# junyanz/interactive-deep-colorization

Hardware: NVIDIA H100
Metric: net_forward images/sec @256x256 (higher is better)
Workload: dtype f16x2-split operands, f32 accumulate (ab within 1e-3 of the f32 reference)

## Files before the change

### interactive_deep_colorization_b200/csrc/idc_api.cu

```cuda
#include <math.h>
#include <stdarg.h>
#include <stdio.h>
#include <string.h>

#include <algorithm>
#include <cmath>

#include "idc_internal.h"

using namespace idc;

struct idc_ctx : public idc::Ctx {};

namespace {

int fail(Ctx* c, int code, const char* fmt, ...) {
  char buf[512];
  va_list ap;
  va_start(ap, fmt);
  vsnprintf(buf, sizeof(buf), fmt, ap);
  va_end(ap);
  if (c) c->err = buf;
  return code;
}
// ... 680 lines not shown
    CUDA_TRY(c, mark());
  }
  const bool fused = !c->simt && !(c->flags & IDC_FLAG_KEEP_CONV10);
  if (!fused) CUDA_TRY(c, launch_out_head(c, n, out_ab, st));
  if (out_dist && !forked) {
    CUDA_TRY(c, launch_softmax529(c, n, out_dist, st));
    CUDA_TRY(c, click_tail(c, n, st));
    pdl_break(c);
  }
  if (out_rgb) {
    CUDA_TRY(c, launch_lab2rgb(c, n, c->H, c->W, L, 50.0f, out_ab, out_rgb, st, out_abq));
    c->launch_count++;
  }
  if (forked) {
    CUDA_TRY(c, cudaStreamWaitEvent(st, c->side->ev_join.get(), 0));
    pdl_break(c);
  }
  CUDA_TRY(c, mark());
  pdl_break(c);
  c->last_n = n;
  return IDC_OK;
}

int check_forward_args(Ctx* c, int n, int h, int w, const void* L, const void* ab, const void* mask, const void* glob,
                       const void* out_ab, const void* out_dist, bool resident_l_ok = false, bool hints_ok = false) {
  if (!c->weights_ready) return fail(c, IDC_ERR_STATE, "idc_forward before idc_finalize_weights");
  if (n < 1 || n > c->max_n) return fail(c, IDC_ERR_ARG, "n=%d outside [1,%d]", n, c->max_n);
  if (h != c->H || w != c->W) return fail(c, IDC_ERR_ARG, "geometry %dx%d != ctx geometry %dx%d", h, w, c->H, c->W);
  const bool hint_mode = hints_ok && !ab && !mask;
  if ((!L && !resident_l_ok) || ((!ab || !mask) && !hint_mode) || !out_ab)
    return fail(c, IDC_ERR_ARG, "null L/ab/mask/out_ab");
  if (out_dist && !c->dist) return fail(c, IDC_ERR_ARG, "out_dist requires IDC_FLAG_DIST");
  if (glob && !c->glob) return fail(c, IDC_ERR_ARG, "glob requires IDC_FLAG_GLOBAL_HINTS");
  return IDC_OK;
}

}

extern "C" {

const char* idc_version(void) { return "idc_b200 0.2 sm_90a (wgmma split-fp16 + fp32 simt engines)"; }

int idc_create(int device, int max_n, int h, int w, unsigned flags, idc_ctx** out) {
  if (!out) return IDC_ERR_ARG;
  *out = nullptr;
  if (max_n < 1 || h < 8 || w < 8 || (h % 8) || (w % 8)) return IDC_ERR_ARG;
  int ndev = 0;
  if (cudaGetDeviceCount(&ndev) != cudaSuccess || device < 0 || device >= ndev) return IDC_ERR_CUDA;
  cudaDeviceProp prop;
  if (cudaGetDeviceProperties(&prop, device) != cudaSuccess) return IDC_ERR_CUDA;
  if (prop.major != 9 || prop.minor != 0) return IDC_ERR_UNSUPPORTED;
  if (cudaSetDevice(device) != cudaSuccess) return IDC_ERR_CUDA;
  std::unique_ptr<idc_ctx> c(new idc_ctx());
  c->dev = device; c->num_sms = prop.multiProcessorCount; c->max_n = max_n; c->H = h; c->W = w; c->flags = flags;
  c->simt = flags & IDC_FLAG_ENGINE_SIMT;
  c->fast = (flags & IDC_FLAG_FAST_FP16) && !c->simt;
  c->dist = flags & IDC_FLAG_DIST;
  c->glob = flags & IDC_FLAG_GLOBAL_HINTS;
  c->caffe313 = flags & IDC_FLAG_CAFFE313;
  build_plan(c.get());
  int rc = alloc_workspace(c.get());
  if (rc != IDC_OK) {
    fprintf(stderr, "idc_create: %s\n", c->err.c_str());
    return rc;
  }
  *out = c.release();
  return IDC_OK;
}

int idc_set_option(idc_ctx* c, const char* name, int value) {
  if (!c || !name) return IDC_ERR_ARG;
  if (!strncmp(name, "act_exp.", 8)) {
    auto it = c->buf_index.find(name + 8);
    if (it == c->buf_index.end() || c->bufs[it->second].H == 0) return fail(c, IDC_ERR_KEY, "no activation '%s'", name + 8);
    if (value < kActExpMin || value > kActExpMax)
      return fail(c, IDC_ERR_ARG, "%s = %d outside [%d, %d]", name, value, kActExpMin, kActExpMax);
    if (c->weights_adopted)
      return fail(c, IDC_ERR_STATE, "%s must be set before the weights are packed (idc_finalize_weights)", name);
    c->act_exp_override[name + 8] = value;
    return IDC_OK;
  }
  struct { const char* n; int* v; } tab[] = {
      {"halo", &c->opt.halo}, {"pairs", &c->opt.pairs}, {"mt", &c->opt.mt},
      {"chunk_kb", &c->opt.chunk_kb}, {"split_k", &c->opt.split_k}, {"host_pipe", &c->opt.host_pipe},
      {"pdl", &c->opt.pdl}, {"tanh_scale", &c->opt.tanh_scale}, {"side_dist", &c->opt.side_dist},
      {"conv1_1_umma", &c->opt.conv1_1_umma}};
  for (auto& t : tab)
    if (!strcmp(t.n, name)) {
      *t.v = value;
      if (c->weights_adopted && strcmp(name, "host_pipe") && strcmp(name, "tanh_scale") && strcmp(name, "side_dist") && strcmp(name, "conv1_1_umma")) {
        CUDA_TRY(c, cudaSetDevice(c->dev));
        CUDA_TRY(c, cudaDeviceSynchronize());
        int rc = plan_engines(c);
        if (rc != IDC_OK) return rc;
      }
      c->graph_exec.reset();
      return IDC_OK;
    }
  return fail(c, IDC_ERR_KEY, "unknown option '%s'", name);
}

int idc_load_tensor(idc_ctx* c, const char* key, const void* data, int dtype, int ndim, const int64_t* dims) {
  if (!c || !key || !data || ndim < 0 || ndim > 8 || (ndim && !dims)) return fail(c, IDC_ERR_ARG, "bad load_tensor args");
  HostTensor t;
  size_t count = 1;
  for (int i = 0; i < ndim; ++i) {
    if (dims[i] < 0) return fail(c, IDC_ERR_ARG, "negative dim");
    t.dims.push_back(dims[i]);
    count *= (size_t)dims[i];
  }
  t.data.resize(count);
  switch (dtype) {
    case IDC_F32: memcpy(t.data.data(), data, count * sizeof(float)); break;
    case IDC_F64: for (size_t i = 0; i < count; ++i) t.data[i] = (float)((const double*)data)[i]; break;
    case IDC_I64: for (size_t i = 0; i < count; ++i) t.data[i] = (float)((const int64_t*)data)[i]; break;
    default: return fail(c, IDC_ERR_ARG, "unknown dtype %d", dtype);
  }
  c->raw[key] = std::move(t);
  c->weights_ready = c->weights_adopted = false;
  return IDC_OK;
}

int idc_reserve_weights(idc_ctx* c) {
  if (!c) return IDC_ERR_ARG;
  CUDA_TRY(c, cudaSetDevice(c->dev));
  if (!c->arena.get()) {
    c->arena_bytes = layout_arena(c, nullptr);
    CUDA_TRY(c, cudaMalloc(c->arena.put(), c->arena_bytes));
    layout_arena(c, c->arena.get());
  }
  return IDC_OK;
}

int idc_finalize_weights(idc_ctx* c) {
  if (!c) return IDC_ERR_ARG;
  int rc = idc_reserve_weights(c);
  if (rc != IDC_OK) return rc;
  std::vector<char> host(c->arena_bytes, 0);
  rc = pack_weights(c, host.data());
  if (rc != IDC_OK) return rc;
  if (c->caffe313) {
    const HostTensor* pts = find(c, "caffe.pts_in_hull");
    if (!check_dims(pts, {313, 2})) return fail(c, IDC_ERR_KEY, "missing/bad caffe.pts_in_hull [313,2]");
    CUDA_TRY(c, cudaMemcpy(c->pts313.get(), pts->data.data(), sizeof(float) * 626, cudaMemcpyHostToDevice));
  }
  CUDA_TRY(c, cudaMemcpy(c->arena.get(), host.data(), c->arena_bytes, cudaMemcpyHostToDevice));
  return idc_adopt_weights(c);
}

int idc_adopt_weights(idc_ctx* c) {
  if (!c || !c->arena.get()) return fail(c, IDC_ERR_STATE, "no arena");
  CUDA_TRY(c, cudaSetDevice(c->dev));
  CUDA_TRY(c, cudaMemcpy(c->h_w11.w, c->w11, sizeof(c->h_w11.w), cudaMemcpyDeviceToHost));
  CUDA_TRY(c, cudaMemcpy(c->h_w11.b, c->b11, sizeof(c->h_w11.b), cudaMemcpyDeviceToHost));
  std::vector<int> exps(c->bufs.size());
  CUDA_TRY(c, cudaMemcpy(exps.data(), c->act_exp, exps.size() * sizeof(int), cudaMemcpyDeviceToHost));
  for (size_t i = 0; i < exps.size(); ++i) c->bufs[i].exp = exps[i];
  if (!c->simt) CUDA_TRY(c, conv1_1_umma_pack(c));
  int rc = plan_engines(c);
  if (rc != IDC_OK) return rc;
  c->raw.clear();
  c->weights_adopted = true;
  c->graph_exec.reset();
  return IDC_OK;
}

int idc_weights_arena(idc_ctx* c, void** dev_ptr, size_t* bytes) {
// ... 799 lines not shown
```

### interactive_deep_colorization_b200/csrc/idc_internal.h

```cpp
#pragma once
#include <cuda.h>
#include <cuda_fp16.h>
#include <cuda_runtime.h>
#include <stdint.h>

#include <map>
#include <memory>
#include <string>
#include <utility>
#include <vector>

#include "../../include/idc_b200.h"

namespace idc {

template <typename H, auto Release>
class Owner {
 public:
  Owner() = default;
  Owner(Owner&& o) noexcept { std::swap(h_, o.h_); }
  Owner& operator=(Owner&& o) noexcept { std::swap(h_, o.h_); return *this; }
  ~Owner() { reset(); }
  H get() const { return h_; }
  H* put() { reset(); return &h_; }
// ... 15 lines not shown

constexpr int kActExpRef = 7;
constexpr int kActExpBound = 11;
constexpr int kActExpCal = 10;
constexpr int kActExpMin = -24, kActExpMax = 24;
constexpr unsigned kRangeInputBit = 31;
constexpr unsigned kF16MaxBits = 0x7BFFu;
constexpr int kInExp = 6;
constexpr float kInScale = 64.0f;

struct Tap {
  int src;
  int ky, kx;
  int ty, tx;
};

struct ActBuf {
  std::string name;
  int H = 0, W = 0, C = 0;
  int exp = 0;
  DevMem<void> p0, p1;
};

struct Epilogue {
  float* bias = nullptr;
  float* scale = nullptr;
  float* shift = nullptr;
  int act = ACT_NONE;
  bool has_bn = false;
  bool gadd = false;
};

struct SrcDesc {
  int buf = -1;
  int s = 1;
  int cin = 0;
};

enum OpKind { OP_CONV = 0, OP_UP = 1, OP_CLASS = 2, OP_HYPER = 3 };

struct UmmaPlan;
struct UmmaPlanFree { void operator()(UmmaPlan* p) const; };

struct ConvOp {
  std::string name;
  int kind = OP_CONV;
  std::string wkey[kMaxSrc];
  bool src_deconv[kMaxSrc] = {false, false, false, false, false, false};
  int src_k[kMaxSrc] = {3, 3, 3, 3, 3, 3};
  std::string bnkey;
  int nsrc = 1;
  SrcDesc src[kMaxSrc];
  int ncls = 1;
  int ntaps = 0;
  Tap taps[kMaxCls][kMaxTaps];
  int Hl = 0, Wl = 0;
  int out_buf = -1;
  int os = 1;
  int cout = 0, cout_pad = 0;
  int K = 0;
  Epilogue epi;
  bool fuse_out_head = false;
  bool out_f32 = false;
  float* out_f32_ptr = nullptr;
  float* w_simt = nullptr;
  __half* w_hi = nullptr;
  __half* w_lo = nullptr;
  int bn_tile = 0, hbox = 0, wbox = 0;
  std::unique_ptr<UmmaPlan, UmmaPlanFree> umma_plan;
  double flops_per_image = 0;
};

struct Conv11Weights {
  float w[36 * 64];
  float b[64];
};

struct Options {
  int halo = 1;
  int pairs = 0;
  int mt = -1;
  int chunk_kb = -1;
  int split_k = -1;
  int host_pipe = 1;
  int pdl = 1;
  int conv1_1_umma = 1;
  int side_dist = 1;
  int tanh_scale = 110;
};

struct HostTensor {
  std::vector<float> data;
  std::vector<int64_t> dims;
};

struct HostStaging {
  DevMem<float> d_in, d_out; HostMem<float> h_in, h_out;
  DevMem<uint8_t> d_rgb; HostMem<uint8_t> h_rgb;
  DevMem<char> d_small; HostMem<char> h_small;
};
struct AbqStaging { DevMem<double> d_abq; HostMem<double> h_abq; };
struct HintBlock { HostMem<char> h_hints; DevMem<char> d_hints; };
struct ClickBlock {
  HostMem<int> h_click; int* d_click = nullptr;
  DevMem<char> d_clickout; HostMem<char> h_clickout;
};
struct SideBranch { Stream s_side, s_click; Event ev_fork, ev_join, ev_click[2]; };
struct HostPipeStreams { Stream s_in, s_out; Event ev_in[8], ev_out[8]; };

struct Ctx {
  int dev = 0;
  int num_sms = 0;
  int max_n = 0, H = 0, W = 0;
  unsigned flags = 0;
  Options opt;
  bool simt = false, fast = false, dist = false, glob = false;
  std::map<std::string, HostTensor> raw;
  std::vector<ActBuf> bufs;
  std::map<std::string, int> buf_index;
  std::vector<ConvOp> ops;
  DevMem<char> arena;
  size_t arena_bytes = 0;
  int* act_exp = nullptr;
  std::map<std::string, int> act_exp_override;
  std::map<std::string, double> act_range;
  DevMem<unsigned> d_absmax;
  bool weights_ready = false;
  bool weights_adopted = false;
  float* w11 = nullptr;
  float* b11 = nullptr;
  Conv11Weights h_w11;
  DevMem<uint8_t> w11_umma;
  float* wout = nullptr;
  float* bout = nullptr;
  float* gw[4] = {nullptr, nullptr, nullptr, nullptr};
  float* gb[4] = {nullptr, nullptr, nullptr, nullptr};
  float* gscale[4] = {nullptr, nullptr, nullptr, nullptr};
  float* gshift[4] = {nullptr, nullptr, nullptr, nullptr};
  DevMem<float> gvec;
  DevMem<float> gtmp;
  DevMem<float> logits;
  DevMem<float> logits313;
  bool caffe313 = false;
  DevMem<float> pts313;
  DevMem<float> splitk_ws; size_t splitk_ws_floats = 0;
  DevMem<int> splitk_counters; int splitk_max_tiles = 0;
  bool dbg_graph_timing = false;
  Event dbg_ev[2];
  float dbg_graph_ms = 0.f;
  HostMem<int> h_err;
  int* d_err = nullptr;
  unsigned* d_range = nullptr;
  std::unique_ptr<HostStaging> stage;
  std::unique_ptr<AbqStaging> abq;
  Stream own_stream;
  std::unique_ptr<HostPipeStreams> pipe;
  std::unique_ptr<SideBranch> side;
  int image_n = 0;
  std::unique_ptr<HintBlock> hints;
  int graph_captures = 0;
  GraphExec graph_exec;
  const void* graph_ptrs[8] = {nullptr};
  float graph_maskcent = 0.f;
  int launch_count = 0;
  int graph_launches = 0;
  bool chain = false;
// ... 209 lines not shown
```

### interactive_deep_colorization_b200/csrc/idc_umma.cu

```cuda
#include <stdio.h>
#include <stdlib.h>

#include "idc_internal.h"

namespace idc {

constexpr int kBM = 128;
constexpr int kBK = 64;
constexpr int kThreads = 384;
constexpr int kProdRegs = 40;
constexpr int kMathRegs = 232;
constexpr int kMathThreads = 256;

struct UmmaParams {
  const CUtensorMap* amaps;
  const int4* kblk;
  int nkb, ncls;
  int chunk_kb;
  int split_k;
  float* ws;
  int* counters;
  int n_img, tiles_y, tiles_x, n_tiles_n, total_tiles;
  int hbox, wbox, wshift;
  int Hl, Wl, cout_pad;
  const float* bias;
  const float* scale;
  const float* shift;
  const float* gadd;
  int gadd_ld;
  float gadd_mult;
  int act;
  __half* out_hi;
  __half* out_lo;
  int Hout, Wout, Cout, os;
  float* out_f32;
  int out_ld;
  const float* wout;
  const float* bout;
  float* out_ab;
  float out_mult;
  int* err;
  unsigned* range;
  unsigned range_bit;
  int n_amaps;
  int max_ctas;
  int img0;
};

__device__ __forceinline__ uint32_t smem_u32(const void* p) { return (uint32_t)__cvta_generic_to_shared(p); }

__device__ __forceinline__ void mbar_init(uint32_t bar, uint32_t count) {
  asm volatile("mbarrier.init.shared::cta.b64 [%0], %1;" ::"r"(bar), "r"(count));
}
__device__ __forceinline__ void mbar_expect_tx(uint32_t bar, uint32_t bytes) {
  asm volatile("mbarrier.arrive.expect_tx.shared::cta.b64 _, [%0], %1;" ::"r"(bar), "r"(bytes) : "memory");
}
__device__ __forceinline__ void mbar_arrive(uint32_t bar) {
  asm volatile("mbarrier.arrive.shared::cta.b64 _, [%0];" ::"r"(bar) : "memory");
}
__device__ __forceinline__ uint32_t mbar_try_wait(uint32_t bar, uint32_t parity) {
  uint32_t ok;
  asm volatile(
      "{\n\t.reg .pred p;\n\t"
      "mbarrier.try_wait.parity.shared::cta.b64 p, [%1], %2;\n\t"
      "selp.u32 %0, 1, 0, p;\n\t}"
      : "=r"(ok)
      : "r"(bar), "r"(parity)
      : "memory");
  return ok;
}
__device__ __noinline__ void mbar_timeout(int* err, int code) {
  if (err) {
    atomicExch(err, code);
    __threadfence_system();
  }
  __trap();
}
__device__ __forceinline__ void mbar_wait(uint32_t bar, uint32_t parity, int* err, int code) {
  if (mbar_try_wait(bar, parity)) return;
  const long long t0 = clock64();
  while (!mbar_try_wait(bar, parity)) {
    if (clock64() - t0 > 6000000000LL) mbar_timeout(err, code);
  }
}

__device__ __forceinline__ bool elect_one() {
  uint32_t pred;
  asm volatile(
      "{\n\t.reg .pred p;\n\t"
      "elect.sync _|p, 0xffffffff;\n\t"
      "selp.u32 %0, 1, 0, p;\n\t}"
      : "=r"(pred));
  return pred != 0;
}

__device__ __forceinline__ void tma_load_4d(uint32_t dst, const void* tmap, uint32_t bar, int c0, int c1, int c2,
                                            int c3) {
  asm volatile(
      "cp.async.bulk.tensor.4d.shared::cluster.global.mbarrier::complete_tx::bytes [%0], [%1, {%3, %4, %5, %6}], [%2];"
      ::"r"(dst), "l"(tmap), "r"(bar), "r"(c0), "r"(c1), "r"(c2), "r"(c3)
      : "memory");
}
__device__ __forceinline__ void tma_load_2d(uint32_t dst, const void* tmap, uint32_t bar, int c0, int c1) {
  asm volatile(
      "cp.async.bulk.tensor.2d.shared::cluster.global.mbarrier::complete_tx::bytes [%0], [%1, {%3, %4}], [%2];"
      ::"r"(dst), "l"(tmap), "r"(bar), "r"(c0), "r"(c1)
      : "memory");
}

__device__ __forceinline__ void tma_load_2d_mc(uint32_t dst, const void* tmap, uint32_t bar, int c0, int c1) {
  asm volatile(
      "cp.async.bulk.tensor.2d.shared::cluster.global.mbarrier::complete_tx::bytes.multicast::cluster"
      " [%0], [%1, {%3, %4}], [%2], %5;"
      ::"r"(dst), "l"(tmap), "r"(bar), "r"(c0), "r"(c1), "h"((uint16_t)3)
      : "memory");
}
__device__ __forceinline__ uint32_t cluster_ctarank() {
  uint32_t r;
  asm volatile("mov.u32 %0, %%cluster_ctarank;" : "=r"(r));
  return r;
}
__device__ __forceinline__ void cluster_sync_all() {
  asm volatile("barrier.cluster.arrive.release.aligned;" ::: "memory");
  asm volatile("barrier.cluster.wait.acquire.aligned;" ::: "memory");
}
__device__ __forceinline__ void mbar_arrive_remote(uint32_t local_bar, uint32_t rank) {
  asm volatile(
      "{\n\t.reg .b32 ra;\n\t"
      "mapa.shared::cluster.u32 ra, %0, %1;\n\t"
      "mbarrier.arrive.release.cluster.shared::cluster.b64 _, [ra];\n\t}"
      ::"r"(local_bar), "r"(rank)
      : "memory");
}

__device__ __forceinline__ void pdl_wait() { asm volatile("griddepcontrol.wait;" ::: "memory"); }
__device__ __forceinline__ void pdl_launch_dependents() { asm volatile("griddepcontrol.launch_dependents;" ::: "memory"); }
__device__ __forceinline__ void prefetch_tmap(const void* tmap) {
  asm volatile("prefetch.tensormap [%0];" ::"l"(tmap) : "memory");
}

__device__ __forceinline__ void st_shared_u32(uint32_t addr, uint32_t v) {
  asm volatile("st.shared.b32 [%0], %1;" ::"r"(addr), "r"(v) : "memory");
}
__device__ __forceinline__ uint4 ld_shared_v4(uint32_t addr) {
  uint4 v;
  asm volatile("ld.shared.v4.b32 {%0, %1, %2, %3}, [%4];" : "=r"(v.x), "=r"(v.y), "=r"(v.z), "=r"(v.w) : "r"(addr));
  return v;
}

__device__ __forceinline__ void wgmma_fence() { asm volatile("wgmma.fence.sync.aligned;" ::: "memory"); }
__device__ __forceinline__ void wgmma_commit() { asm volatile("wgmma.commit_group.sync.aligned;" ::: "memory"); }
template <int N>
__device__ __forceinline__ void wgmma_wait() { asm volatile("wgmma.wait_group.sync.aligned %0;" ::"n"(N) : "memory"); }
template <int R>
__device__ __forceinline__ void wgmma_reg_fence(float (&d)[R]) {
#pragma unroll
  for (int i = 0; i < R; ++i) asm volatile("" : "+f"(d[i])::"memory");
}

__device__ __forceinline__ void wgmma_n64(float (&d)[32], uint64_t adesc, uint64_t bdesc, uint32_t accumulate) {
  asm volatile(
      "{\n\t.reg .pred p;\n\t"
      "setp.ne.b32 p, %34, 0;\n\t"
      "wgmma.mma_async.sync.aligned.m64n64k16.f32.f16.f16 "
// ... 19 lines not shown
  if constexpr (BN == 128) wgmma_n128(d, adesc, bdesc, accumulate);
  else wgmma_n64(d, adesc, bdesc, accumulate);
}

__device__ __forceinline__ uint64_t make_sw128_desc(uint32_t smem_addr, uint32_t sbo = 1024u) {
  uint64_t d = 0;
  d |= (uint64_t)((smem_addr >> 4) & 0x3FFFu);
  d |= (uint64_t)1 << 16;
  d |= (uint64_t)(sbo >> 4) << 32;
  d |= (uint64_t)1 << 62;
  return d;
}

__device__ __forceinline__ uint32_t pack_f16x2_sat(float a, float b) {
  uint32_t r;
  asm("cvt.rn.satfinite.f16x2.f32 %0, %1, %2;" : "=r"(r) : "f"(b), "f"(a));
  return r;
}
__device__ __forceinline__ uint32_t lo_f16x2(float a, float b, uint32_t hw) {
  const float2 hf = __half22float2(*reinterpret_cast<const __half2*>(&hw));
  return pack_f16x2_sat(a - hf.x, b - hf.y);
}
__device__ __forceinline__ uint32_t habs_max2(uint32_t m, uint32_t w) {
  const __half2 r = __hmax2(*reinterpret_cast<const __half2*>(&m), __habs2(*reinterpret_cast<const __half2*>(&w)));
  return *reinterpret_cast<const uint32_t*>(&r);
}
__device__ __forceinline__ bool f16_top(uint32_t m) {
  return ((m & 0xFFFFu) >= kF16MaxBits) | ((m >> 16) >= kF16MaxBits);
}

__device__ __forceinline__ void split_h(float v, __half& hi, __half& lo) {
  v = fminf(fmaxf(v, -65504.f), 65504.f);
  hi = __float2half_rn(v);
  lo = __float2half_rn(v - __half2float(hi));
}

__device__ __forceinline__ int frag_col(int i, int lane) { return 8 * (i >> 2) + 2 * (lane & 3) + (i & 1); }

constexpr int kHaloW = 10, kHaloH = 18;
constexpr int kHaloPlane = (kHaloW * kHaloH * 128 + 1023) / 1024 * 1024;


template <int BN, int MT, int CG, bool SPLIT, bool HALO>
struct SmemPlan {
  static constexpr int kABytes = MT * kBM * kBK * 2;
  static constexpr int kAStage = HALO ? 0 : kABytes;
  static constexpr int kBBytes = BN * kBK * 2;
  static constexpr int kStageBytes = (SPLIT ? 2 : 1) * (kAStage + kBBytes);
  static constexpr int kHaloSlot = (SPLIT ? 2 : 1) * kHaloPlane;
  static constexpr int kHaloBytes = HALO ? 2 * kHaloSlot : 0;
  static constexpr int kOutRow = 64 * 2 + 16;
  static constexpr int kOutWarp = 16 * kOutRow;
  static constexpr int kOutStage = 8 * kOutWarp;
  static constexpr int kTail = 3 * BN * 4 + 272 * 4 + 256;
  static constexpr int kBudget = 232448 - 1024 - kTail - kOutStage - kHaloBytes;
  static constexpr int kStages = kBudget / kStageBytes >= 4 ? 4 : kBudget / kStageBytes;
  static constexpr int kTotal = kStages * kStageBytes + kHaloBytes + kOutStage + kTail + 1024;
  static_assert(kStages >= 2, "need at least a double-buffered operand ring");
  static_assert(MT * BN <= 128, "register budget: chunk + tile accumulators of MT*BN columns per math thread pair");
  static_assert(!HALO || MT == 1, "halo tiles are single 16x8-pixel M-tiles");
  static_assert(CG == 1 || CG == 2, "clusters of one or two CTAs");
};

template <int BN, int MT, int CG, bool SPLIT, bool HALO>
__global__ void __launch_bounds__(kThreads, 1)
umma_conv_kernel(const __grid_constant__ CUtensorMap bmap_hi, const __grid_constant__ CUtensorMap bmap_lo,
                 const __grid_constant__ UmmaParams p) {
  using SP = SmemPlan<BN, MT, CG, SPLIT, HALO>;
  constexpr int STAGES = SP::kStages;
  constexpr int R = BN / 2;
  constexpr bool PAIR = CG == 2;
  extern __shared__ uint8_t smem_raw[];
  uint8_t* smem = reinterpret_cast<uint8_t*>((reinterpret_cast<uintptr_t>(smem_raw) + 1023) & ~uintptr_t(1023));
  uint8_t* s_halo = smem + STAGES * SP::kStageBytes;
  uint8_t* s_out = s_halo + SP::kHaloBytes;
  float* s_bias = reinterpret_cast<float*>(s_out + SP::kOutStage);
  float* s_scale = s_bias + BN;
  float* s_shift = s_scale + BN;
  float* s_head = s_shift + BN;
  uint64_t* full_bar = reinterpret_cast<uint64_t*>(s_head + 272);
  uint64_t* empty_bar = full_bar + 4;
  uint64_t* afull_bar = full_bar + 8;
  uint64_t* aempty_bar = full_bar + 10;

  const int warp = threadIdx.x >> 5, lane = threadIdx.x & 31;
  const uint32_t cta_rank = PAIR ? cluster_ctarank() : 0u;

  if (p.wout) {
    for (int i = threadIdx.x; i < 256; i += kThreads) s_head[i] = p.wout[i];
    if (threadIdx.x < 2) s_head[256 + threadIdx.x] = p.bout[threadIdx.x];
  }
  if (threadIdx.x == 32) {
    prefetch_tmap(&bmap_hi);
    if (SPLIT) prefetch_tmap(&bmap_lo);
    for (int i = 0; i < p.n_amaps; ++i) prefetch_tmap(p.amaps + i);
  }
  if (threadIdx.x == 0) {
    for (int s = 0; s < STAGES; ++s) {
      mbar_init(smem_u32(&full_bar[s]), 1);
      mbar_init(smem_u32(&empty_bar[s]), 8 * CG);
    }
    if (HALO)
      for (int a = 0; a < 2; ++a) {
        mbar_init(smem_u32(&afull_bar[a]), 1);
        mbar_init(smem_u32(&aempty_bar[a]), 8);
      }
    asm volatile("fence.mbarrier_init.release.cluster;" ::: "memory");
  }
  if (PAIR) cluster_sync_all(); else __syncthreads();
  pdl_launch_dependents();
  pdl_wait();

  const int tiles_per_img = p.tiles_y * p.tiles_x;
  const int S = p.split_k;
  const int n_items = p.total_tiles * S;
  const int w0 = blockIdx.x / CG, wstep = gridDim.x / CG;

  if (warp < 4) {
    asm volatile("setmaxnreg.dec.sync.aligned.u32 %0;" ::"n"(kProdRegs));
    if (warp == 0) {
      int stage = 0;
      uint32_t phase = 0;
      uint32_t hcount = 0;
      for (int w = w0; w < n_items; w += wstep) {
        const int tile = w / S, ks = w - tile * S;
        const int kbeg = (ks * p.nkb) / S, kend = ((ks + 1) * p.nkb) / S;
        int r = tile;
        const int nt = r % p.n_tiles_n;
        r /= p.n_tiles_n;
        const int cls = r % p.ncls;
        r /= p.ncls;
        if (PAIR) r = 2 * r + (int)cta_rank;
        const int img_rel = r / tiles_per_img;
        r -= img_rel * tiles_per_img;
        const int img = p.img0 + img_rel;
        const int y0 = (r / p.tiles_x) * (p.hbox * MT), x0 = (r % p.tiles_x) * p.wbox;
        const int brow = cls * p.cout_pad + nt * BN + (int)cta_rank * (BN / CG);
        const int4* kb = p.kblk + cls * p.nkb;
        for (int k = kbeg; k < kend; ++k) {
          if (HALO && k % 9 == 0) {
            const uint32_t slot = hcount & 1, hphase = (hcount >> 1) & 1;
            ++hcount;
            mbar_wait(smem_u32(&aempty_bar[slot]), hphase ^ 1, p.err, 6);
            if (elect_one()) {
              const uint32_t fa = smem_u32(&afull_bar[slot]);
              const uint32_t sh = smem_u32(s_halo + slot * SP::kHaloSlot);
              const int c0 = (k / 9) * kBK;
              mbar_expect_tx(fa, (SPLIT ? 2 : 1) * kHaloW * kHaloH * 128);
              tma_load_4d(sh, p.amaps, fa, c0, x0 - 1, y0 - 1, img);
              if (SPLIT) tma_load_4d(sh + kHaloPlane, p.amaps + 1, fa, c0, x0 - 1, y0 - 1, img);
            }
            __syncwarp();
          }
          mbar_wait(smem_u32(&empty_bar[stage]), phase ^ 1, p.err, 1);
          if (elect_one()) {
            const uint32_t fb = smem_u32(&full_bar[stage]);
            const int4 e = __ldg(kb + k);
            const uint32_t sa = smem_u32(smem + stage * SP::kStageBytes);
            const uint32_t sb = sa + (SPLIT ? 2 : 1) * SP::kAStage + cta_rank * (BN / CG) * 128;
            const int kcol = HALO ? e.y : k * kBK;
            mbar_expect_tx(fb, SP::kStageBytes);
            if (!HALO) {
              const CUtensorMap* am = p.amaps + e.x;
              tma_load_4d(sa, am, fb, e.y, x0 + e.w, y0 + e.z, img);
              if (SPLIT) tma_load_4d(sa + SP::kABytes, am + 1, fb, e.y, x0 + e.w, y0 + e.z, img);
            }
            if (PAIR) {
              tma_load_2d_mc(sb, &bmap_hi, fb, kcol, brow);
              if (SPLIT) tma_load_2d_mc(sb + SP::kBBytes, &bmap_lo, fb, kcol, brow);
            } else {
              tma_load_2d(sb, &bmap_hi, fb, kcol, brow);
              if (SPLIT) tma_load_2d(sb + SP::kBBytes, &bmap_lo, fb, kcol, brow);
            }
          }
          __syncwarp();
          if (++stage == STAGES) { stage = 0; phase ^= 1; }
        }
      }
    }
  } else {
    asm volatile("setmaxnreg.inc.sync.aligned.u32 %0;" ::"n"(kMathRegs));
    const int et = threadIdx.x - 128;
    const int wg = et >> 7;
    const int wi = (et >> 5) & 3;
    const uint32_t wbuf = smem_u32(s_out) + (uint32_t)(et >> 5) * SP::kOutWarp;
    auto release = [&](uint64_t* bar) {
      __syncwarp();
      if (lane == 0) {
        mbar_arrive(smem_u32(bar));
        if (PAIR) mbar_arrive_remote(smem_u32(bar), cta_rank ^ 1u);
      }
    };
    int stage = 0;
    uint32_t phase = 0;
    uint32_t hcount = 0;
    int staged_key = -1;
    bool sat = false;
    for (int w = w0; w < n_items; w += wstep) {
      const int tile = w / S, ks = w - tile * S;
      const int kbeg = (ks * p.nkb) / S, kend = ((ks + 1) * p.nkb) / S;
      int r = tile;
      const int nt = r % p.n_tiles_n;
      r /= p.n_tiles_n;
      const int cls = r % p.ncls;
      r /= p.ncls;
      if (PAIR) r = 2 * r + (int)cta_rank;
      const int img_rel = r / tiles_per_img;
      r -= img_rel * tiles_per_img;
      const int img = p.img0 + img_rel;
      const int ty0 = (r / p.tiles_x) * (p.hbox * MT), tx0 = (r % p.tiles_x) * p.wbox;
      const int n0 = nt * BN;
      const int vkey = p.gadd ? (img * p.n_tiles_n + nt) : nt;
      if (vkey != staged_key) {
        asm volatile("bar.sync 1, 256;" ::: "memory");
        for (int i = et; i < BN; i += kMathThreads) {
          s_bias[i] = p.bias[n0 + i];
          s_scale[i] = p.scale[n0 + i];
          const int gi = img < p.n_img ? img : p.n_img - 1;
          s_shift[i] = p.shift[n0 + i] + (p.gadd ? p.gadd[(size_t)gi * p.gadd_ld + n0 + i] * p.gadd_mult : 0.f);
        }
        asm volatile("bar.sync 1, 256;" ::: "memory");
        staged_key = vkey;
      }

      float acc[MT][R];
#pragma unroll
      for (int m = 0; m < MT; ++m)
#pragma unroll
        for (int j = 0; j < R; ++j) acc[m][j] = 0.f;
      for (int k0 = kbeg; k0 < kend; k0 += p.chunk_kb) {
        const int k1 = (k0 + p.chunk_kb < kend) ? k0 + p.chunk_kb : kend;
        float part[MT][R];
#pragma unroll
        for (int m = 0; m < MT; ++m)
#pragma unroll
          for (int j = 0; j < R; ++j) part[m][j] = 0.f;
        int prev = -1;
        for (int k = k0; k < k1; ++k) {
          uint32_t hslot = 0;
          if (HALO) {
            if (k % 9 == 0) {
              mbar_wait(smem_u32(&afull_bar[hcount & 1]), (hcount >> 1) & 1, p.err, 7);
              ++hcount;
            }
            hslot = (hcount - 1) & 1;
          }
          mbar_wait(smem_u32(&full_bar[stage]), phase, p.err, 3);
          const uint32_t st0 = smem_u32(smem + stage * SP::kStageBytes);
          const uint32_t sb = st0 + (SPLIT ? 2 : 1) * SP::kAStage;
          const uint64_t b_hi = make_sw128_desc(sb), b_lo = make_sw128_desc(sb + SP::kBBytes);
          uint32_t ha = 0;
          if (HALO) {
            const int4 e = __ldg(p.kblk + k);
            ha = smem_u32(s_halo + hslot * SP::kHaloSlot) + (uint32_t)((e.z + wg * 8) * kHaloW + e.w) * 128u;
          }
          wgmma_fence();
#pragma unroll
          for (int m = 0; m < MT; ++m) {
            const uint32_t sa = st0 + (uint32_t)(wg * MT + m) * (64 * 128);
            const uint64_t a_hi = HALO ? make_sw128_desc(ha, kHaloW * 128) : make_sw128_desc(sa);
            const uint64_t a_lo = HALO ? make_sw128_desc(ha + kHaloPlane, kHaloW * 128) : make_sw128_desc(sa + SP::kABytes);
            uint32_t first = (k == k0) ? 0u : 1u;
            if (SPLIT) {
#pragma unroll
              for (int kk = 0; kk < kBK / 16; ++kk) {
                const uint64_t adv = (uint64_t)(kk * 2);
                wgmma_bn<BN>(part[m], a_lo + adv, b_hi + adv, first);
                wgmma_bn<BN>(part[m], a_hi + adv, b_lo + adv, 1u);
                first = 1u;
              }
            }
#pragma unroll
            for (int kk = 0; kk < kBK / 16; ++kk) {
              const uint64_t adv = (uint64_t)(kk * 2);
              wgmma_bn<BN>(part[m], a_hi + adv, b_hi + adv, first);
              first = 1u;
            }
          }
          wgmma_commit();
          if (HALO && k % 9 == 8) {
            wgmma_wait<0>();
            __syncwarp();
            if (lane == 0) mbar_arrive(smem_u32(&aempty_bar[hslot]));
          }
          if (prev >= 0) {
            wgmma_wait<1>();
            release(&empty_bar[prev]);
          }
          prev = stage;
          if (++stage == STAGES) { stage = 0; phase ^= 1; }
        }
        wgmma_wait<0>();
#pragma unroll
        for (int m = 0; m < MT; ++m) wgmma_reg_fence(part[m]);
        release(&empty_bar[prev]);
#pragma unroll
        for (int m = 0; m < MT; ++m)
#pragma unroll
          for (int j = 0; j < R; ++j) acc[m][j] += part[m][j];
      }

      if (S > 1) {
        float* wp = p.ws + (size_t)w * R * kMathThreads + et;
#pragma unroll
        for (int i = 0; i < R; ++i)
          if ((i >> 4) % S != ks) __stcg(wp + (size_t)i * kMathThreads, acc[0][i]);
        __threadfence();
        asm volatile("bar.sync 1, 256;" ::: "memory");
        if (et == 0) {
          int* cnt = p.counters + 2 * tile;
          atomicAdd(cnt, 1);
          const long long t0 = clock64();
          int seen;
          do {
            asm volatile("ld.acquire.gpu.global.s32 %0, [%1];" : "=r"(seen) : "l"(cnt) : "memory");
            if (seen < S && clock64() - t0 > 6000000000LL) mbar_timeout(p.err, 5);
          } while (seen < S);
        }
        asm volatile("bar.sync 1, 256;" ::: "memory");
        for (int q = 0; q < S; ++q) {
          if (q == ks) continue;
          const float* rp = p.ws + (size_t)(tile * S + q) * R * kMathThreads + et;
#pragma unroll
          for (int i = 0; i < R; ++i)
            if ((i >> 4) % S == ks) acc[0][i] += __ldcg(rp + (size_t)i * kMathThreads);
        }
      }

      const float neg_slope = p.act == ACT_RELU ? 0.f : (p.act == ACT_LEAKY02 ? 0.2f : 1.f);
      unsigned own = ~0u;
      if (S > 1) {
        own = 0u;
#pragma unroll
        for (int pc = 0; pc < BN / 32; ++pc) own |= (pc % S == ks ? 1u : 0u) << pc;
      }
#pragma unroll
      for (int m = 0; m < MT; ++m) {
        const int blk = (wg * MT + m) * 64;
#pragma unroll
        for (int i = 0; i < R; ++i) {
          const int c = frag_col(i, lane);
          const float t = acc[m][i] + s_bias[c];
          acc[m][i] = fmaf(fmaxf(t, neg_slope * t), s_scale[c], s_shift[c]);
        }
        int ry[2], rx[2];
        bool ok[2];
#pragma unroll
        for (int h = 0; h < 2; ++h) {
          const int rr = blk + wi * 16 + (lane >> 2) + 8 * h;
          ry[h] = ty0 + (rr >> p.wshift);
          rx[h] = tx0 + (rr & (p.wbox - 1));
          ok[h] = ry[h] < p.Hl && rx[h] < p.Wl && img < p.n_img;
        }
        if (p.wout) {
          float h0[2] = {0.f, 0.f}, h1[2] = {0.f, 0.f};
#pragma unroll
          for (int i = 0; i < R; ++i) {
            const int c = frag_col(i, lane), h = (i >> 1) & 1;
            h0[h] = fmaf(acc[m][i], s_head[c], h0[h]);
            h1[h] = fmaf(acc[m][i], s_head[128 + c], h1[h]);
          }
#pragma unroll
          for (int h = 0; h < 2; ++h) {
#pragma unroll
            for (int o = 1; o <= 2; o <<= 1) {
              h0[h] += __shfl_xor_sync(0xffffffffu, h0[h], o);
              h1[h] += __shfl_xor_sync(0xffffffffu, h1[h], o);
            }
            if ((lane & 3) == 0 && ok[h]) {
              const size_t HW = (size_t)p.Hl * p.Wl;
              const size_t o = (size_t)img * 2 * HW + (size_t)ry[h] * p.Wl + rx[h];
              p.out_ab[o] = tanhf(h0[h] + s_head[256]) * p.out_mult;
              p.out_ab[o + HW] = tanhf(h1[h] + s_head[257]) * p.out_mult;
            }
          }
        } else if (p.out_f32) {
#pragma unroll
          for (int i = 0; i < R; i += 2) {
            const int h = (i >> 1) & 1;
            if ((S > 1 && (i >> 4) % S != ks) || !ok[h]) continue;
            float* o = p.out_f32 + ((size_t)(img * p.Hl + ry[h]) * p.Wl + rx[h]) * p.out_ld + n0 + frag_col(i, lane);
            *reinterpret_cast<float2*>(o) = make_float2(acc[m][i], acc[m][i + 1]);
          }
        } else {
          __half* prow[4];
          const int rl0 = lane >> 3, ch = lane & 7;
#pragma unroll
          for (int it = 0; it < 4; ++it) {
            const int rr = blk + wi * 16 + rl0 + 4 * it;
            const int yy = ty0 + (rr >> p.wshift), xx = tx0 + (rr & (p.wbox - 1));
            const bool v = yy < p.Hl && xx < p.Wl && img < p.n_img;
            prow[it] = v ? p.out_hi + ((size_t)(img * p.Hout + yy * p.os + (cls >> 1)) * p.Wout + xx * p.os + (cls & 1)) * p.Cout +
                               n0 + ch * 8
                         : nullptr;
          }
          const ptrdiff_t lo_delta = SPLIT ? p.out_lo - p.out_hi : 0;
          uint32_t hmax[2][BN / 32] = {};
#pragma unroll
          for (int sl = 0; sl < BN / 64; ++sl) {
            if (S > 1 && ((2 * sl) % S != ks) && ((2 * sl + 1) % S != ks)) continue;
#pragma unroll
            for (int plane = 0; plane < (SPLIT ? 2 : 1); ++plane) {
#pragma unroll
              for (int i = 32 * sl; i < 32 * sl + 32; i += 2) {
                const uint32_t hw = pack_f16x2_sat(acc[m][i], acc[m][i + 1]);
                if (plane == 0) hmax[(i >> 1) & 1][i >> 4] = habs_max2(hmax[(i >> 1) & 1][i >> 4], hw);
                const uint32_t v = plane == 0 ? hw : lo_f16x2(acc[m][i], acc[m][i + 1], hw);
                const int rl = (lane >> 2) + 8 * ((i >> 1) & 1), cl = frag_col(i, lane) - 64 * sl;
                st_shared_u32(wbuf + rl * SP::kOutRow + cl * 2, v);
              }
              __syncwarp();
#pragma unroll
              for (int it = 0; it < 4; ++it) {
                const uint4 v = ld_shared_v4(wbuf + (rl0 + 4 * it) * SP::kOutRow + ch * 16);
                const int piece = (64 * sl + ch * 8) >> 5;
                if (prow[it] && (S == 1 || piece % S == ks))
                  *reinterpret_cast<uint4*>(prow[it] + (plane ? lo_delta : 0) + 64 * sl) = v;
              }
              __syncwarp();
            }
          }
          uint32_t top = 0u;
#pragma unroll
          for (int pc = 0; pc < BN / 32; ++pc) {
            const bool mine = (own >> pc) & 1u;
            top = habs_max2(top, (mine & ok[0]) ? hmax[0][pc] : 0u);
            top = habs_max2(top, (mine & ok[1]) ? hmax[1][pc] : 0u);
          }
          sat |= f16_top(top);
        }
      }
      if (S > 1) {
        asm volatile("bar.sync 1, 256;" ::: "memory");
        if (et == 0) {
          int* cnt = p.counters + 2 * tile;
          if (atomicAdd(cnt + 1, 1) == S - 1) { cnt[0] = 0; cnt[1] = 0; __threadfence(); }
        }
      }
    }
    if (__any_sync(0xffffffffu, sat) && lane == 0) atomicOr(p.range, p.range_bit);
  }
  if (PAIR) cluster_sync_all();
}

constexpr int kC11K = 48;
constexpr int kC11PackBytes = 2 * 8192 + 2 * 64 * 4;
constexpr int kC11Smem = 2 * 16384 + kC11PackBytes + 1024;

__device__ __forceinline__ uint32_t sw128_off(int row, int chunk) {
  return (uint32_t)((row >> 3) * 1024 + (row & 7) * 128 + ((chunk ^ (row & 7)) << 4));
}

__global__ void conv1_1_pack_kernel(const float* __restrict__ w36x64, const float* __restrict__ bias, int s_out,
                                    uint8_t* __restrict__ out) {
  const int co = threadIdx.x;
  if (co >= 64) return;
  float mx = 0.f;
  for (int k = 0; k < 36; ++k) mx = fmaxf(mx, fabsf(w36x64[k * 64 + co]));
  int e = 0;
  if (mx > 0.f) { int ex; frexpf(mx, &ex); e = 9 - ex; }
  const float sc = ldexpf(1.f, e);
  __half* bh = reinterpret_cast<__half*>(out);
  __half* bl = reinterpret_cast<__half*>(out + 8192);
  for (int k = 0; k < 64; ++k) {
    const float v = k < 36 ? w36x64[k * 64 + co] * sc : 0.f;
    __half hi, lo;
    split_h(v, hi, lo);
    const uint32_t o = (sw128_off(co, k >> 3) >> 1) + (k & 7);
    bh[o] = hi; bl[o] = lo;
  }
  float* vec = reinterpret_cast<float*>(out + 16384);
  vec[co] = bias[co] * kInScale * sc;
  vec[64 + co] = ldexpf(1.f, s_out - kInExp - e);
}

template <bool SPLIT>
__global__ void __launch_bounds__(128, 4)
conv1_1_umma_kernel(const uint8_t* __restrict__ pack, const float* __restrict__ L, const float* __restrict__ ab,
                    const float* __restrict__ mask, float maskcent, int N, int H, int Wd, __half* __restrict__ ohi,
                    __half* __restrict__ olo, unsigned* range, unsigned out_bit) {
  extern __shared__ uint8_t smem_raw[];
  uint8_t* smem = reinterpret_cast<uint8_t*>((reinterpret_cast<uintptr_t>(smem_raw) + 1023) & ~uintptr_t(1023));
  uint8_t* s_ahi = smem;
  uint8_t* s_alo = smem + 16384;
  uint8_t* s_pack = smem + 32768;
  const float* s_vec = reinterpret_cast<const float*>(s_pack + 16384);
  const int warp = threadIdx.x >> 5, lane = threadIdx.x & 31;
  constexpr int kRow = 64 * 2 + 16;

  {
    const uint4* src = reinterpret_cast<const uint4*>(pack);
    uint4* dst = reinterpret_cast<uint4*>(s_pack);
    for (int i = threadIdx.x; i < kC11PackBytes / 16; i += 128) dst[i] = __ldg(src + i);
  }
  asm volatile("fence.proxy.async.shared::cta;" ::: "memory");
  __syncthreads();
  pdl_launch_dependents();
  pdl_wait();

  const size_t HW = (size_t)H * Wd, total = (size_t)N * HW;
  const int ntiles = (int)((total + 127) / 128);
  for (int tile = blockIdx.x; tile < ntiles; tile += gridDim.x) {
    const size_t pix = (size_t)tile * 128 + threadIdx.x;
    const bool live = pix < total;
    const size_t pixc = live ? pix : 0;
    const int n = (int)(pixc / HW);
    const int r = (int)(pixc - (size_t)n * HW);
    const int y = r / Wd, x = r - y * Wd;
    float in[kC11K];
#pragma unroll
    for (int ky = 0; ky < 3; ++ky)
#pragma unroll
      for (int kx = 0; kx < 3; ++kx) {
        const int iy = y + ky - 1, ix = x + kx - 1;
        const bool ok = live && iy >= 0 && iy < H && ix >= 0 && ix < Wd;
        const size_t o = (size_t)iy * Wd + ix;
        const int t = (ky * 3 + kx) * 4;
        const float l = ok ? __ldg(L + (size_t)n * HW + o) : 0.f;
        const float a = ok ? __ldg(ab + (size_t)n * 2 * HW + o) : 0.f;
        const float b = ok ? __ldg(ab + (size_t)n * 2 * HW + HW + o) : 0.f;
        const float m = ok ? __ldg(mask + (size_t)n * HW + o) - maskcent : 0.f;
        const float ql = l * 0.01f, qa = a * (1.0f / 110.0f), qb = b * (1.0f / 110.0f);
// ... 294 lines not shown
      const int g = i / 9, t = i % 9;
      kblk[i] = make_int4(0, (t * groups + g) * kBK, op.taps[0][t].ty + 1, op.taps[0][t].tx + 1);
    }
  }
  for (int cls = 0; cls < op.ncls && !pl->halo; ++cls) {
    int kb = 0;
    for (int t = 0; t < op.ntaps; ++t) {
      const Tap& tp = op.taps[cls][t];
      const int s = op.src[tp.src].s;
      ViewKey vk{tp.src, s, 0, 0};
      int dy = tp.ty, dx = tp.tx;
      if (s == 2) {
        vk.qy = ((tp.ty % 2) + 2) % 2; vk.qx = ((tp.tx % 2) + 2) % 2;
        dy = floordiv2(tp.ty); dx = floordiv2(tp.tx);
      }
      int vi = -1;
      for (size_t i = 0; i < views.size(); ++i)
        if (views[i] == vk) vi = (int)i;
      if (vi < 0) { views.push_back(vk); vi = (int)views.size() - 1; }
      const int cin = op.src[tp.src].cin;
      if (cin % kBK) { c->err = "cin not a multiple of 64: " + op.name; return IDC_ERR_ARG; }
      for (int c0 = 0; c0 < cin; c0 += kBK) kblk[(size_t)cls * nkb + kb++] = make_int4(vi * 2, c0, dy, dx);
    }
    if (kb != nkb) { c->err = "k-block count mismatch: " + op.name; return IDC_ERR_ARG; }
  }
  std::vector<CUtensorMap> amaps(views.size() * 2);
  for (size_t i = 0; i < views.size(); ++i) {
    const ViewKey& vk = views[i];
    const ActBuf& b = c->bufs[op.src[vk.src].buf];
    const int Hv = (b.H - vk.qy + vk.s - 1) / vk.s, Wv = (b.W - vk.qx + vk.s - 1) / vk.s;
    for (int part = 0; part < 2; ++part) {
      char* base = (char*)(part == 0 ? b.p0.get() : b.p1.get());
      if (!base) { amaps[i * 2 + part] = amaps[i * 2]; continue; }
      base += ((size_t)vk.qy * b.W + vk.qx) * b.C * sizeof(__half);
      cuuint64_t dims[4] = {(cuuint64_t)b.C, (cuuint64_t)Wv, (cuuint64_t)Hv, (cuuint64_t)c->max_n};
      cuuint64_t strides[3] = {(cuuint64_t)vk.s * b.C * 2, (cuuint64_t)vk.s * b.W * b.C * 2,
                               (cuuint64_t)b.H * b.W * b.C * 2};
      cuuint32_t box[4] = {(cuuint32_t)kBK, (cuuint32_t)(pl->halo ? kHaloW : op.wbox),
                           (cuuint32_t)(pl->halo ? kHaloH : op.hbox * pl->mt), 1};
      cuuint32_t estr[4] = {1, 1, 1, 1};
      CUresult r = enc(&amaps[i * 2 + part], CU_TENSOR_MAP_DATA_TYPE_FLOAT16, 4, base, dims, strides, box, estr,
                       CU_TENSOR_MAP_INTERLEAVE_NONE, CU_TENSOR_MAP_SWIZZLE_128B, CU_TENSOR_MAP_L2_PROMOTION_L2_128B,
                       CU_TENSOR_MAP_FLOAT_OOB_FILL_NONE);
      if (r != CUDA_SUCCESS) {
        char msg[256];
        snprintf(msg, sizeof(msg), "cuTensorMapEncodeTiled(A) failed (%d) for op %s view %zu", (int)r, op.name.c_str(), i);
        c->err = msg;
        return IDC_ERR_CUDA;
      }
    }
  }
  for (int part = 0; part < 2; ++part) {
    cuuint64_t dims[2] = {(cuuint64_t)op.K, (cuuint64_t)op.ncls * op.cout_pad};
    cuuint64_t strides[1] = {(cuuint64_t)op.K * 2};
    cuuint32_t box[2] = {(cuuint32_t)kBK, (cuuint32_t)(op.bn_tile / pl->cg)};
    cuuint32_t estr[2] = {1, 1};
    CUresult r = enc(part == 0 ? &pl->bmap_hi : &pl->bmap_lo, CU_TENSOR_MAP_DATA_TYPE_FLOAT16, 2,
                     part == 0 ? (void*)op.w_hi : (void*)op.w_lo, dims, strides, box, estr,
                     CU_TENSOR_MAP_INTERLEAVE_NONE, CU_TENSOR_MAP_SWIZZLE_128B, CU_TENSOR_MAP_L2_PROMOTION_L2_256B,
                     CU_TENSOR_MAP_FLOAT_OOB_FILL_NONE);
    if (r != CUDA_SUCCESS) {
      char msg[256];
      snprintf(msg, sizeof(msg), "cuTensorMapEncodeTiled(B) failed (%d) for op %s", (int)r, op.name.c_str());
      c->err = msg;
      return IDC_ERR_CUDA;
    }
  }
  if (cudaMalloc(pl->d_amaps.put(), amaps.size() * sizeof(CUtensorMap)) != cudaSuccess ||
      cudaMalloc(pl->d_kblk.put(), kblk.size() * sizeof(int4)) != cudaSuccess ||
      cudaMemcpy(pl->d_amaps.get(), amaps.data(), amaps.size() * sizeof(CUtensorMap), cudaMemcpyHostToDevice) != cudaSuccess ||
      cudaMemcpy(pl->d_kblk.get(), kblk.data(), kblk.size() * sizeof(int4), cudaMemcpyHostToDevice) != cudaSuccess) {
    c->err = "uploading the launch plan failed in umma_plan_op: " + op.name;
    return IDC_ERR_CUDA;
  }

  UmmaParams& q = pl->prm;
  q.amaps = pl->d_amaps.get(); q.n_amaps = (int)amaps.size(); q.kblk = pl->d_kblk.get(); q.nkb = nkb; q.ncls = op.ncls;
  {
    const int natural = (op.cout_pad % 256 == 0) ? 256 : (op.cout_pad % 192 == 0) ? 192 : (op.cout_pad % 128 == 0) ? 128 : 64;
    int g = c->fast ? 4 : (natural <= 128 ? 2 : 1);
    if (c->opt.chunk_kb >= 1) g = c->opt.chunk_kb;
    q.chunk_kb = g;
  }
  q.tiles_y = ceil_div(op.Hl, op.hbox * pl->mt); q.tiles_x = ceil_div(op.Wl, op.wbox);
  q.n_tiles_n = op.cout_pad / op.bn_tile;
  q.hbox = op.hbox; q.wbox = op.wbox;
  q.wshift = 0;
  while ((1 << q.wshift) < op.wbox) q.wshift++;
  q.Hl = op.Hl; q.Wl = op.Wl; q.cout_pad = op.cout_pad;
  q.bias = op.epi.bias; q.scale = op.epi.scale; q.shift = op.epi.shift;
  q.gadd = nullptr; q.gadd_ld = 512; q.gadd_mult = op.out_buf >= 0 ? ldexpf(1.f, c->bufs[op.out_buf].exp) : 1.f;
  q.act = op.epi.act;
  if (op.out_f32) {
    q.out_f32 = op.out_f32_ptr; q.out_ld = op.cout_pad;
  } else if (op.out_buf >= 0) {
    const ActBuf& ob = c->bufs[op.out_buf];
    q.out_hi = (__half*)ob.p0.get(); q.out_lo = (__half*)ob.p1.get();
    q.Hout = ob.H; q.Wout = ob.W; q.Cout = ob.C; q.os = op.os;
  }
  if (op.fuse_out_head) { q.wout = c->wout; q.bout = c->bout; }
  q.err = c->d_err;
  q.range = c->d_range; q.range_bit = op.out_buf >= 0 ? 1u << op.out_buf : 0u;
  q.img0 = 0;
  op.umma_plan = std::move(pl);
  return IDC_OK;
}

void UmmaPlanFree::operator()(UmmaPlan* p) const { delete p; }

bool umma_op_uses_split_k(const ConvOp& op) {
  return op.umma_plan && op.umma_plan->split_k > 1;
}

cudaError_t umma_run_op(Ctx* c, ConvOp& op, int n, float* out_ab_fused, float out_mult, cudaStream_t st, int img0,
                        int max_ctas) {
  const UmmaPlan* pl = op.umma_plan.get();
  if (!pl) return cudaErrorInvalidValue;
  UmmaParams prm = pl->prm;
  prm.max_ctas = (max_ctas > 0 && pl->split_k == 1) ? (max_ctas / pl->cg) * pl->cg : 0;
  prm.img0 = img0;
  prm.n_img = img0 + n;
  if (img0 && pl->split_k > 1) return cudaErrorInvalidValue;
  const int m_tiles = n * prm.tiles_y * prm.tiles_x;
  prm.total_tiles = op.ncls * (pl->cg == 2 ? (m_tiles + 1) / 2 : m_tiles) * prm.n_tiles_n;
  prm.gadd = (op.epi.gadd && c->gadd_active) ? c->gvec.get() : nullptr;
  prm.out_ab = out_ab_fused;
  prm.split_k = pl->split_k;
  prm.ws = c->splitk_ws.get();
  prm.counters = c->splitk_counters.get();
  if (pl->split_k > 1 && (!prm.ws || !prm.counters)) return cudaErrorInvalidValue;
  prm.out_mult = out_mult;
  if (op.fuse_out_head && !out_ab_fused) return cudaErrorInvalidValue;
  c->launch_count++;
  const bool pdl = pdl_take(c);
  const bool split = !c->fast;
  if (pl->halo) {
    if (!split) return cudaErrorInvalidValue;
    switch (op.bn_tile * 10 + pl->cg) {
      case 641: return launch_inst<64, 1, 1, true, true>(*pl, prm, st, pdl);
      case 642: return launch_inst<64, 1, 2, true, true>(*pl, prm, st, pdl);
      case 1281: return launch_inst<128, 1, 1, true, true>(*pl, prm, st, pdl);
      case 1282: return launch_inst<128, 1, 2, true, true>(*pl, prm, st, pdl);
      default: return cudaErrorInvalidValue;
    }
  }
#define IDC_LAUNCH(BN_, MT_, CG_) \
  return split ? launch_inst<BN_, MT_, CG_, true>(*pl, prm, st, pdl) : launch_inst<BN_, MT_, CG_, false>(*pl, prm, st, pdl)
  switch (op.bn_tile * 100 + pl->mt * 10 + pl->cg) {
    case 6411: IDC_LAUNCH(64, 1, 1);
    case 6421: IDC_LAUNCH(64, 2, 1);
    case 12811: IDC_LAUNCH(128, 1, 1);
    case 6412: return launch_inst<64, 1, 2, true>(*pl, prm, st, pdl);
    case 6422: return launch_inst<64, 2, 2, true>(*pl, prm, st, pdl);
    case 12812: return launch_inst<128, 1, 2, true>(*pl, prm, st, pdl);
    default: break;
  }
#undef IDC_LAUNCH
  return cudaErrorInvalidValue;
}

}
```

Baseline: 1363.

## Add ping-pong turn barriers between math warpgroups and defer halo slot release

Adds a pair of mbarriers that pass a turn token between the two math warpgroups, so one group's WGMMA issue overlaps the other's epilogue in a ping-pong schedule. By default this is enabled for non-fast, single-class ops, and the handoff point inside the last k-block can be tuned through a new option. The halo slot release is also moved after the wgmma_wait<1> of the next iteration, which removes the blocking wgmma_wait<0> on every ninth k-block. The cost is extra barrier traffic and the risk of serialising the warpgroups or deadlocking when the turn counts do not match.

```diff
diff --git a/interactive_deep_colorization_b200/csrc/idc_api.cu b/interactive_deep_colorization_b200/csrc/idc_api.cu
--- a/interactive_deep_colorization_b200/csrc/idc_api.cu
+++ b/interactive_deep_colorization_b200/csrc/idc_api.cu
@@ -786,7 +786,8 @@
   }
   struct { const char* n; int* v; } tab[] = {
       {"halo", &c->opt.halo}, {"pairs", &c->opt.pairs}, {"mt", &c->opt.mt},
-      {"chunk_kb", &c->opt.chunk_kb}, {"split_k", &c->opt.split_k}, {"host_pipe", &c->opt.host_pipe},
+      {"chunk_kb", &c->opt.chunk_kb}, {"split_k", &c->opt.split_k}, {"wg_turns", &c->opt.wg_turns},
+      {"host_pipe", &c->opt.host_pipe},
       {"pdl", &c->opt.pdl}, {"tanh_scale", &c->opt.tanh_scale}, {"side_dist", &c->opt.side_dist},
       {"conv1_1_umma", &c->opt.conv1_1_umma}};
   for (auto& t : tab)
diff --git a/interactive_deep_colorization_b200/csrc/idc_internal.h b/interactive_deep_colorization_b200/csrc/idc_internal.h
--- a/interactive_deep_colorization_b200/csrc/idc_internal.h
+++ b/interactive_deep_colorization_b200/csrc/idc_internal.h
@@ -121,6 +121,7 @@
   int mt = -1;
   int chunk_kb = -1;
   int split_k = -1;
+  int wg_turns = -1;
   int host_pipe = 1;
   int pdl = 1;
   int conv1_1_umma = 1;
diff --git a/interactive_deep_colorization_b200/csrc/idc_umma.cu b/interactive_deep_colorization_b200/csrc/idc_umma.cu
--- a/interactive_deep_colorization_b200/csrc/idc_umma.cu
+++ b/interactive_deep_colorization_b200/csrc/idc_umma.cu
@@ -45,6 +45,7 @@
   int n_amaps;
   int max_ctas;
   int img0;
+  int wg_turns;
 };
 
 __device__ __forceinline__ uint32_t smem_u32(const void* p) { return (uint32_t)__cvta_generic_to_shared(p); }
@@ -80,6 +81,17 @@
   if (mbar_try_wait(bar, parity)) return;
   const long long t0 = clock64();
   while (!mbar_try_wait(bar, parity)) {
+    if (clock64() - t0 > 6000000000LL) mbar_timeout(err, code);
+  }
+}
+__device__ __forceinline__ void mbar_arrive_lane0(uint32_t bar, int lane) {
+  asm volatile("{\n\t.reg .pred p;\n\tsetp.eq.s32 p, %1, 0;\n\t@p mbarrier.arrive.shared::cta.b64 _, [%0];\n\t}"
+               ::"r"(bar), "r"(lane) : "memory");
+}
+__device__ __forceinline__ void mbar_wait_warp(uint32_t bar, uint32_t parity, int* err, int code) {
+  if (__all_sync(0xffffffffu, mbar_try_wait(bar, parity))) return;
+  const long long t0 = clock64();
+  while (!__all_sync(0xffffffffu, mbar_try_wait(bar, parity))) {
     if (clock64() - t0 > 6000000000LL) mbar_timeout(err, code);
   }
 }
@@ -265,6 +277,7 @@
   uint64_t* empty_bar = full_bar + 4;
   uint64_t* afull_bar = full_bar + 8;
   uint64_t* aempty_bar = full_bar + 10;
+  uint64_t* turn_bar = full_bar + 12;
 
   const int warp = threadIdx.x >> 5, lane = threadIdx.x & 31;
   const uint32_t cta_rank = PAIR ? cluster_ctarank() : 0u;
@@ -288,6 +301,9 @@
         mbar_init(smem_u32(&afull_bar[a]), 1);
         mbar_init(smem_u32(&aempty_bar[a]), 8);
       }
+    for (int g = 0; g < 2; ++g) mbar_init(smem_u32(&turn_bar[g]), 4);
+    if (p.wg_turns)
+      for (int i = 0; i < 4; ++i) mbar_arrive(smem_u32(&turn_bar[0]));
     asm volatile("fence.mbarrier_init.release.cluster;" ::: "memory");
   }
   if (PAIR) cluster_sync_all(); else __syncthreads();
@@ -374,6 +390,12 @@
         if (PAIR) mbar_arrive_remote(smem_u32(bar), cta_rank ^ 1u);
       }
     };
+    auto release_halo = [&](int slot) {
+      __syncwarp();
+      if (lane == 0) mbar_arrive(smem_u32(&aempty_bar[slot]));
+    };
+    const uint32_t turn_in = smem_u32(&turn_bar[wg]), turn_out = smem_u32(&turn_bar[wg ^ 1]);
+    uint32_t turns = 0;
     int stage = 0;
     uint32_t phase = 0;
     uint32_t hcount = 0;
@@ -418,7 +440,9 @@
         for (int m = 0; m < MT; ++m)
 #pragma unroll
           for (int j = 0; j < R; ++j) part[m][j] = 0.f;
+        if (p.wg_turns) mbar_wait_warp(turn_in, turns & 1, p.err, 8);
         int prev = -1;
+        int hpend = -1;
         for (int k = k0; k < k1; ++k) {
           uint32_t hslot = 0;
           if (HALO) {
@@ -437,6 +461,7 @@
             const int4 e = __ldg(p.kblk + k);
             ha = smem_u32(s_halo + hslot * SP::kHaloSlot) + (uint32_t)((e.z + wg * 8) * kHaloW + e.w) * 128u;
           }
+          const int pass_at = (k == k1 - 1) ? p.wg_turns : 0;
           wgmma_fence();
 #pragma unroll
           for (int m = 0; m < MT; ++m) {
@@ -451,6 +476,7 @@
                 wgmma_bn<BN>(part[m], a_lo + adv, b_hi + adv, first);
                 wgmma_bn<BN>(part[m], a_hi + adv, b_lo + adv, 1u);
                 first = 1u;
+                if (m == 0 && pass_at == kk + 2) mbar_arrive_lane0(turn_out, lane);
               }
             }
 #pragma unroll
@@ -461,22 +487,23 @@
             }
           }
           wgmma_commit();
-          if (HALO && k % 9 == 8) {
-            wgmma_wait<0>();
-            __syncwarp();
-            if (lane == 0) mbar_arrive(smem_u32(&aempty_bar[hslot]));
-          }
+          if (pass_at && !(SPLIT && pass_at >= 2)) mbar_arrive_lane0(turn_out, lane);
           if (prev >= 0) {
             wgmma_wait<1>();
             release(&empty_bar[prev]);
+            if (HALO && hpend >= 0) release_halo(hpend);
+            hpend = -1;
           }
+          if (HALO && k % 9 == 8) hpend = (int)hslot;
           prev = stage;
           if (++stage == STAGES) { stage = 0; phase ^= 1; }
         }
+        ++turns;
         wgmma_wait<0>();
 #pragma unroll
         for (int m = 0; m < MT; ++m) wgmma_reg_fence(part[m]);
         release(&empty_bar[prev]);
+        if (HALO && hpend >= 0) release_halo(hpend);
 #pragma unroll
         for (int m = 0; m < MT; ++m)
 #pragma unroll
@@ -621,6 +648,7 @@
         }
       }
     }
+    if (p.wg_turns && wg == 0) mbar_wait(turn_in, turns & 1, p.err, 8);
     if (__any_sync(0xffffffffu, sat) && lane == 0) atomicOr(p.range, p.range_bit);
   }
   if (PAIR) cluster_sync_all();
@@ -1081,6 +1109,7 @@
     if (c->opt.chunk_kb >= 1) g = c->opt.chunk_kb;
     q.chunk_kb = g;
   }
+  q.wg_turns = c->opt.wg_turns < 0 ? ((!c->fast && op.ncls == 1) ? 4 : 0) : (c->opt.wg_turns > 5 ? 5 : c->opt.wg_turns);
   q.tiles_y = ceil_div(op.Hl, op.hbox * pl->mt); q.tiles_x = ceil_div(op.Wl, op.wbox);
   q.n_tiles_n = op.cout_pad / op.bn_tile;
   q.hbox = op.hbox; q.wbox = op.wbox;
```

Measured after the change: 1371, median of 6. Within noise of the previous version (+0.6%).
